# razvanmatisan/duodiff

Hardware: AMD Instinct MI355X
Metric: images/sec (whole node) DuoDiff 1000-step CelebA-64 (higher is better)
Workload: dtype bf16

## Files before the change

duodiff_amd/csrc/attention.hip:

```cpp
#include "dd_internal.h"

#include <type_traits>
#include <utility>

namespace dd {
namespace {

constexpr int kMaxKeyTiles = 9;
constexpr int kLP = kMaxKeyTiles * 32;
constexpr int kHD = 64;
constexpr int kPartBytes = 4 * 2 * 66 * 4;

__device__ __forceinline__ unsigned pack2_bf16(float lo, float hi) {
    typedef __bf16 bf16v2 __attribute__((ext_vector_type(2)));
    typedef float f32v2 __attribute__((ext_vector_type(2)));
    const f32v2 q = {lo, hi};
    return __builtin_bit_cast(unsigned, __builtin_convertvector(q, bf16v2));
}

__device__ __forceinline__ unsigned lds_addr_of(const void* p) {
    return (unsigned)(size_t)(const __attribute__((address_space(3))) char*)p;
}

__device__ __forceinline__ int k_swz(int r) { return ((r >> 1) & 7) ^ ((r & 1) << 2); }
__device__ __forceinline__ int v_swz(int r) { return (2 * (r & 3)) ^ ((r >> 2) & 1); }

template <typename T> struct AttnLayout;
template <> struct AttnLayout<bf16_t> {
    static constexpr int kRowK = 128;
    static constexpr int kRowV = 128;
    static constexpr int kVBytes = kLP * kRowV;
};
template <> struct AttnLayout<float> {
    static constexpr int kRowK = 256 + 16;
    static constexpr int kRowV = kLP * 4 + 16;
    static constexpr int kVBytes = kHD * kRowV;
};

template <typename T, int NKT, int NT, bool KPERM, typename TileFn>
__device__ __forceinline__ void attend_tiles(const char* Ks, const char* Vt, int L, int nkt, int lane, TileFn&& tile,
                                         const f32x4 (&qcur)[sizeof(T) == 2 ? 4 : 8], f32x16 (&o)[2], float& mx, float& sum) {
    using Lay = AttnLayout<T>;
    const int half = lane >> 5, r32 = lane & 31;
    const f32x16 zero16 = {0.f, 0.f, 0.f, 0.f, 0.f, 0.f, 0.f, 0.f, 0.f, 0.f, 0.f, 0.f, 0.f, 0.f, 0.f, 0.f};
    f32x16 s[NT];

    if constexpr (sizeof(T) == 2) {
        bf16x8 qf[4];
#pragma unroll
        for (int st = 0; st < 4; ++st) qf[st] = __builtin_bit_cast(bf16x8, qcur[st]);
        auto load_k = [&](int t, bf16x8 (&kf)[4]) {
            const char* kr = Ks + (t * 32 + r32) * Lay::kRowK;
            const int sw = k_swz(r32);
#pragma unroll
            for (int st = 0; st < 4; ++st) {
                const int ch = KPERM ? 4 * (st >> 1) + 2 * half + (st & 1) : 2 * st + half;
                kf[st] = *reinterpret_cast<const bf16x8*>(kr + ((ch ^ sw) << 4));
            }
        };
        bf16x8 kfa[4], kfb[4];
        if (tile(0) >= 0) load_k(tile(0), kfa);
#pragma unroll
        for (int k = 0; k < NT; ++k) {
            const int t = tile(k);
            const int tn = k + 1 < NT ? tile(k + 1) : -1;
            if (tn >= 0) { if (k & 1) load_k(tn, kfa); else load_k(tn, kfb); }
            __builtin_amdgcn_sched_barrier(0);
            if (t >= 0) {
                s[k] = __builtin_amdgcn_mfma_f32_32x32x16_bf16((k & 1) ? kfb[0] : kfa[0], qf[0], zero16, 0, 0, 0);
#pragma unroll
                for (int st = 1; st < 4; ++st)
                    s[k] = __builtin_amdgcn_mfma_f32_32x32x16_bf16((k & 1) ? kfb[st] : kfa[st], qf[st], s[k], 0, 0, 0);
            } else {
                s[k] = zero16;
            }
            __builtin_amdgcn_sched_barrier(0);
        }
    } else {
#pragma unroll
        for (int k = 0; k < NT; ++k) {
            const int t = tile(k);
            s[k] = zero16;
            if (t >= 0) {
                const char* kr = Ks + (t * 32 + r32) * Lay::kRowK + (32 * half) * 4;
#pragma unroll
                for (int g = 0; g < 8; ++g) {
                    const f32x4 kf = *reinterpret_cast<const f32x4*>(kr + g * 16);
#pragma unroll
                    for (int e = 0; e < 4; ++e)
                        s[k] = __builtin_amdgcn_mfma_f32_32x32x2f32(kf[e], qcur[g][e], s[k], 0, 0, 0);
                }
            }
        }
    }

    mx = -INFINITY;
#pragma unroll
    for (int k = 0; k < NT; ++k) {
        const int t = tile(k);
        if (t >= 0) {
            if (t == nkt - 1) {
#pragma unroll
                for (int e = 0; e < 16; ++e) {
                    const int key = t * 32 + (e & 3) + 8 * (e >> 2) + 4 * half;
                    if (key >= L) s[k][e] = -INFINITY;
                }
            }
#pragma unroll
            for (int e = 0; e < 16; ++e) mx = fmaxf(mx, s[k][e]);
        }
    }
    mx = fmaxf(mx, __shfl_xor(mx, 32));
    constexpr float kScaleLog2e = 0.125f * 1.4426950408889634f;
    const float mxs = mx * kScaleLog2e;
    sum = 0.f;
#pragma unroll
    for (int k = 0; k < NT; ++k) {
        if (tile(k) >= 0) {
#pragma unroll
            for (int e = 0; e < 16; ++e) {
                float p;
                if (NKT == 9 && NT == 9 && k == 8 && e >= 2) {
                    s[k][e] = 0.f;
                    continue;
                }
                if constexpr (sizeof(T) == 2) p = __builtin_amdgcn_exp2f(fmaf(s[k][e], kScaleLog2e, -mxs));
                else p = expf((s[k][e] - mx) * 0.125f);
                s[k][e] = p;
                sum += p;
            }
        }
    }
    sum += __shfl_xor(sum, 32);

    o[0] = zero16;
    o[1] = zero16;

    if constexpr (sizeof(T) == 2) {
        typedef __attribute__((ext_vector_type(4))) short s4;
        struct VF { s4 lo[2][2], hi[2][2]; };
        const int tq = (lane >> 2) & 3, tp = lane & 3, dhalf = (lane >> 4) & 1;
        const char* vb0 = Vt + (4 * half + tq) * Lay::kRowV + 8 * (tp & 1);
        const int vsw = v_swz(4 * half + tq);
        const char* vbd[2] = {vb0 + (((2 * dhalf + (tp >> 1)) ^ vsw) << 4), vb0 + (((4 + 2 * dhalf + (tp >> 1)) ^ vsw) << 4)};
        typedef __attribute__((address_space(3))) s4* lds_s4_ptr;
        auto load_v = [&](int t, VF& f) {
#pragma unroll
            for (int st = 0; st < 2; ++st)
#pragma unroll
                for (int dt = 0; dt < 2; ++dt) {
                    const char* vr = vbd[dt] + (t * 32 + 16 * st) * Lay::kRowV;
                    f.lo[st][dt] = __builtin_amdgcn_ds_read_tr16_b64_v4i16((lds_s4_ptr)(size_t)lds_addr_of(vr));
                    f.hi[st][dt] = __builtin_amdgcn_ds_read_tr16_b64_v4i16((lds_s4_ptr)(size_t)lds_addr_of(vr + 8 * Lay::kRowV));
                }
        };
        VF va, vb;
        if (tile(0) >= 0) load_v(tile(0), va);
#pragma unroll
        for (int k = 0; k < NT; ++k) {
            const int t = tile(k);
            const int tn = k + 1 < NT ? tile(k + 1) : -1;
            if (tn >= 0) { if (k & 1) load_v(tn, va); else load_v(tn, vb); }
            __builtin_amdgcn_sched_barrier(0);
            if (t >= 0) {
                const VF& f = (k & 1) ? vb : va;
#pragma unroll
                for (int st = 0; st < 2; ++st) {
                    bf16x8 pf;
#pragma unroll
                    for (int j = 0; j < 8; ++j) pf[j] = (short)f2bf(s[k][8 * st + j]);
#pragma unroll
                    for (int dt = 0; dt < 2; ++dt) {
                        bf16x8 vf;
#pragma unroll
                        for (int j = 0; j < 4; ++j) { vf[j] = f.lo[st][dt][j]; vf[4 + j] = f.hi[st][dt][j]; }
                        o[dt] = __builtin_amdgcn_mfma_f32_32x32x16_bf16(vf, pf, o[dt], 0, 0, 0);
                    }
                }
            }
            __builtin_amdgcn_sched_barrier(0);
        }
    } else {
#pragma unroll
        for (int k = 0; k < NT; ++k) {
            const int t = tile(k);
            if (t >= 0) {
#pragma unroll
                for (int g = 0; g < 4; ++g) {
#pragma unroll
                    for (int dt = 0; dt < 2; ++dt) {
                        const char* vr = Vt + (dt * 32 + r32) * Lay::kRowV + (t * 32 + 8 * g + 4 * half) * 4;
                        const f32x4 vf = *reinterpret_cast<const f32x4*>(vr);
#pragma unroll
                        for (int e = 0; e < 4; ++e)
                            o[dt] = __builtin_amdgcn_mfma_f32_32x32x2f32(vf[e], s[k][4 * g + e], o[dt], 0, 0, 0);
                    }
                }
            }
        }
    }
}

template <typename T, int NKT>
__global__ void __launch_bounds__(256, sizeof(T) == 2 ? 2 : 1)
attention_kernel(const T* __restrict__ qkv, T* __restrict__ out, int B, int L, int H, int D, int Lp) {
    using Lay = AttnLayout<T>;
    extern __shared__ __attribute__((aligned(16))) char smem[];
    char* Ks = smem;
    char* Vt = smem + kLP * Lay::kRowK;

    const int b = blockIdx.x / H, hh = blockIdx.x % H;
    const int tid = threadIdx.x, lane = tid & 63, wave = tid >> 6;
    const int half = lane >> 5, r32 = lane & 31;
    constexpr long long ld = kHD;
    const long long unit = (long long)Lp * kHD;
    const T* qbase = qkv + ((long long)b * 3 * H + hh) * unit;
    const T* kbase = qbase + (long long)H * unit;
    const T* vbase = kbase + (long long)H * unit;
    const int nkt = NKT > 0 ? NKT : (L + 31) / 32;
    constexpr int EPC = 16 / (int)sizeof(T);
    constexpr int CPR = kHD / EPC;

    constexpr int NQF = sizeof(T) == 2 ? 4 : 8;
    auto load_q = [&](int qc, f32x4 (&qf)[NQF]) {
        const int q = qc * 32 + r32;
        const T* qrow = qbase + (long long)(q < L ? q : L - 1) * ld;
#pragma unroll
        for (int i = 0; i < NQF; ++i)
            qf[i] = sizeof(T) == 2 ? *reinterpret_cast<const f32x4*>(qrow + 16 * i + 8 * half)
                                   : *reinterpret_cast<const f32x4*>(qrow + 32 * half + 4 * i);
    };
    f32x4 qnext[NQF];
    load_q(wave, qnext);

    if constexpr (sizeof(T) == 2) {
        typedef const __attribute__((address_space(1))) void* gptr_t;
        typedef __attribute__((address_space(3))) void* lptr_t;
        const int np = Lp >> 3;
        const int wv = __builtin_amdgcn_readfirstlane(wave);
        const int lr = lane >> 3, slot = lane & 7;
        constexpr int MAXP = (kLP / 8 * 2 + 3) / 4;
#pragma unroll
        for (int i = 0; i < MAXP; ++i) {
            const int p2 = wv + 4 * i;
            if (p2 < 2 * np) {
                const bool isv = p2 >= np;
                const int p = isv ? p2 - np : p2, r = 8 * p + lr;
                const int ch = isv ? (slot ^ v_swz(r)) : (slot ^ k_swz(r));
                const T* src = (isv ? vbase : kbase) + (long long)(r < L ? r : L - 1) * kHD + ch * 8;
                char* dst = (isv ? Vt : Ks) + p * 1024;
                __builtin_amdgcn_global_load_lds((gptr_t)src, (lptr_t)dst, 16, 0, 0);
            }
        }
        for (int i = tid; i < (nkt * 32 - Lp) * 16; i += 256) {
            const int rr = Lp + (i >> 4), c = i & 15;
            *reinterpret_cast<f32x4*>((c < 8 ? Ks : Vt) + rr * 128 + (c & 7) * 16) = f32x4{0.f, 0.f, 0.f, 0.f};
        }
        asm volatile("s_waitcnt vmcnt(0)" ::: "memory");
    } else {
        for (int idx = tid; idx < nkt * 32 * CPR; idx += 256) {
            const int key = idx / CPR, ch = idx % CPR;
            f32x4 kv = {0.f, 0.f, 0.f, 0.f}, vv = {0.f, 0.f, 0.f, 0.f};
            if (key < L) {
                kv = *reinterpret_cast<const f32x4*>(kbase + (long long)key * ld + ch * EPC);
                vv = *reinterpret_cast<const f32x4*>(vbase + (long long)key * ld + ch * EPC);
            }
            *reinterpret_cast<f32x4*>(Ks + key * Lay::kRowK + ch * 16) = kv;
            T tmp[EPC];
            *reinterpret_cast<f32x4*>(tmp) = vv;
#pragma unroll
            for (int e = 0; e < EPC; ++e)
                *reinterpret_cast<T*>(Vt + (ch * EPC + e) * Lay::kRowV + key * (int)sizeof(T)) = tmp[e];
        }
    }

    __syncthreads();

    constexpr bool SPLIT_LAST = NKT == 9;
    const int nqc = (L + 31) / 32;
    const int n_regular = SPLIT_LAST ? 8 : nqc;
    for (int qc = wave; qc < n_regular; qc += 4) {
        const int q = qc * 32 + r32;
        f32x4 qcur[NQF];
#pragma unroll
        for (int i = 0; i < NQF; ++i) qcur[i] = qnext[i];
        if (qc + 4 < n_regular) load_q(qc + 4, qnext);
        else if (SPLIT_LAST) load_q(8, qnext);

        f32x16 o[2];
        float mx, sum;
        attend_tiles<T, NKT, kMaxKeyTiles, false>(Ks, Vt, L, nkt, lane, [&](int k) { return k < nkt ? k : -1; }, qcur, o, mx, sum);
        const float inv = 1.0f / sum;

        T* orow = out + ((long long)b * L + (q < L ? q : L - 1)) * D + hh * kHD;
        if constexpr (sizeof(T) == 2) {
#pragma unroll
            for (int dt = 0; dt < 2; ++dt) {
                uint2 v[4];
#pragma unroll
                for (int g = 0; g < 4; ++g) {
                    bf16_t v4[4];
#pragma unroll
                    for (int e = 0; e < 4; ++e) v4[e] = f2bf(o[dt][4 * g + e] * inv);
                    v[g] = *reinterpret_cast<const uint2*>(v4);
                }
#pragma unroll
                for (int gp = 0; gp < 4; gp += 2) {
                    const auto s0 = __builtin_amdgcn_permlane32_swap(v[gp].x, v[gp + 1].x, false, false);
                    const auto s1 = __builtin_amdgcn_permlane32_swap(v[gp].y, v[gp + 1].y, false, false);
                    const uint4 o4 = {s0[0], s1[0], s0[1], s1[1]};
                    if (q < L) *reinterpret_cast<uint4*>(orow + dt * 32 + 8 * gp + 8 * half) = o4;
                }
            }
        } else if (q < L) {
#pragma unroll
            for (int dt = 0; dt < 2; ++dt)
#pragma unroll
                for (int g = 0; g < 4; ++g) {
                    const int d = dt * 32 + 8 * g + 4 * half;
                    *reinterpret_cast<f32x4*>(orow + d) = f32x4{o[dt][4 * g] * inv, o[dt][4 * g + 1] * inv, o[dt][4 * g + 2] * inv, o[dt][4 * g + 3] * inv};
                }
        }
    }

    if constexpr (SPLIT_LAST) {
        float* part = reinterpret_cast<float*>(smem + kLP * Lay::kRowK + Lay::kVBytes);
        const int rem = L - 256;
        f32x16 o[2];
        float mx, sum;
        attend_tiles<T, NKT, 3, false>(Ks, Vt, L, nkt, lane, [&](int k) { return k < 2 ? wave + 4 * k : (wave == 3 ? 8 : -1); }, qnext, o, mx, sum);
        if (r32 < rem) {
            float* pw = part + (wave * 2 + r32) * 66;
#pragma unroll
            for (int dt = 0; dt < 2; ++dt)
#pragma unroll
                for (int g = 0; g < 4; ++g)
                    *reinterpret_cast<f32x4*>(pw + dt * 32 + 8 * g + 4 * half) =
                        f32x4{o[dt][4 * g], o[dt][4 * g + 1], o[dt][4 * g + 2], o[dt][4 * g + 3]};
            if (half == 0) { pw[64] = mx; pw[65] = sum; }
        }
        __syncthreads();
        if (tid < rem * 64) {
            const int qi = tid >> 6, d = tid & 63;
            float m[4], M = -INFINITY;
#pragma unroll
            for (int w = 0; w < 4; ++w) { m[w] = part[(w * 2 + qi) * 66 + 64]; M = fmaxf(M, m[w]); }
            float num = 0.f, den = 0.f;
#pragma unroll
            for (int w = 0; w < 4; ++w) {
                float f;
                if constexpr (sizeof(T) == 2) f = __builtin_amdgcn_exp2f((m[w] - M) * (0.125f * 1.4426950408889634f));
                else f = expf((m[w] - M) * 0.125f);
                num = fmaf(f, part[(w * 2 + qi) * 66 + d], num);
                den = fmaf(f, part[(w * 2 + qi) * 66 + 65], den);
            }
            out[((long long)b * L + 256 + qi) * D + hh * kHD + d] = Elem<T>::from_f32(num / den);
        }
    }
}


struct QkvAttnArgs {
    const bf16_t* h;
    const bf16_t* wimg;
    const float* bias;
    const bf16_t* hx;
    const float* xres;
    const float* ln_g;
    const float* ln_b;
    bf16_t* out;
    int B, L, H, Lp, E;
};

constexpr int kQaPxBytes = 8 * 6 * 2 * 32 * 4;
constexpr int kQaHxPad = 64;
constexpr int kQaHxBytes = 2 * (1024 * 2 + kQaHxPad);
constexpr int kQaAuxBytes = kQaPxBytes + kQaHxBytes + 256;
constexpr int kQaKQ = 8;
constexpr int kQaBlk = 2 * kQaKQ * 1024;
constexpr int kQaRing = 4 * kQaBlk;
static_assert(8 * 2 * 66 * 4 <= kQaPxBytes, "the split chunk's partials reuse the px area");

typedef const __attribute__((address_space(1))) void* qa_gptr_t;
typedef __attribute__((address_space(3))) void* qa_lptr_t;

constexpr int qa_dma_ops(int b, int nb) { return b < nb ? 2 : 0; }
constexpr int qa_pref_ops(int b, int nb) { return (b >= 0 && b % 3 == 0 && b / 3 + 1 < nb / 3) ? kQaKQ : 0; }
constexpr int qa_younger_dma(int b, int nb) { return qa_pref_ops(b - 1, nb) + qa_dma_ops(b + 2, nb) + qa_pref_ops(b, nb); }
constexpr int qa_younger_rows(int b, int nb) { return qa_dma_ops(b, nb) + qa_dma_ops(b + 1, nb) + qa_dma_ops(b + 2, nb); }

template <int D>
__global__ void __launch_bounds__(512, 1) qkv_attention_kernel(const QkvAttnArgs a) {
    using Lay = AttnLayout<bf16_t>;
    constexpr int KS = D / 16, NS = KS / kQaKQ, NB = 3 * NS;
    static_assert(D % 128 == 0 && D >= 512 && D <= 1024, "k range in slices of 8 k-steps; hxl holds two rows of D <= 1024");
    extern __shared__ __attribute__((aligned(16))) char smem[];
    char* Ks = smem;
    char* Vt = smem + kLP * Lay::kRowK;
    float* px = reinterpret_cast<float*>(smem + kLP * Lay::kRowK + Lay::kVBytes);
    float* part = px;
    char* hxl = smem + kLP * Lay::kRowK + Lay::kVBytes + kQaPxBytes;
    char* qxl = hxl + kQaHxBytes;
    char* ring = smem + kLP * Lay::kRowK + Lay::kVBytes + kQaAuxBytes;

    int b, hh;
    if ((a.B & 7) == 0) { const int slot = blockIdx.x >> 3; b = (blockIdx.x & 7) + 8 * (slot / a.H); hh = slot % a.H; }
    else { b = blockIdx.x / a.H; hh = blockIdx.x % a.H; }
    const int tid = threadIdx.x, lane = tid & 63, wave = __builtin_amdgcn_readfirstlane(tid >> 6);
    const int half = lane >> 5, r32 = lane & 31;
    const int L = a.L, E = a.E;

    const char* wsrc = reinterpret_cast<const char*>(a.wimg) + (size_t)hh * NB * kQaBlk;
    const unsigned lane16 = lane * 16;
    auto dma_block = [&](int bb) {
#pragma unroll
        for (int i = 0; i < 2; ++i) {
            const int pc = wave * 2 + i;
            const char* sb = wsrc + (size_t)bb * kQaBlk + pc * 1024;
            const unsigned lds = lds_addr_of(ring + (bb & 3) * kQaBlk + pc * 1024);
            asm volatile("s_mov_b32 m0, %0\n\tglobal_load_lds_dwordx4 %1, %2" ::"s"(lds), "v"(lane16), "s"(sb) : "memory", "m0");
        }
    };
    dma_block(0);
    dma_block(1);
    dma_block(2);

    const int row = 32 * wave + r32;
    const bf16x8* hfr_u = reinterpret_cast<const bf16x8*>(a.h) + ((long long)b * 8 + wave) * KS * 64;
    const bf16x8* hfr = hfr_u + lane;
    bf16x8 xs[2][kQaKQ];
#pragma unroll
    for (int ks = 0; ks < kQaKQ; ++ks) xs[0][ks] = hfr[ks * 64];

    if (a.hx) {
        for (int i = tid; i < E * (D / 8); i += 512) {
            const int e = i / (D / 8), cch = i % (D / 8);
            *reinterpret_cast<f32x4*>(hxl + e * (D * 2 + kQaHxPad) + cch * 16) = *reinterpret_cast<const f32x4*>(a.hx + ((long long)b * L + e) * D + cch * 8);
        }
    } else if (wave < E) {
        constexpr int NV = D / 256;
        const float* xr = a.xres + ((long long)b * L + wave) * D + lane * (D / 64);
        f32x4 xv[NV];
        float s1 = 0.f;
#pragma unroll
        for (int v = 0; v < NV; ++v) {
            xv[v] = *reinterpret_cast<const f32x4*>(xr + 4 * v);
            s1 += (xv[v][0] + xv[v][1]) + (xv[v][2] + xv[v][3]);
        }
#pragma unroll
        for (int o = 32; o >= 1; o >>= 1) s1 += __shfl_xor(s1, o);
        const float mean = s1 / (float)D;
        float s2 = 0.f;
#pragma unroll
        for (int v = 0; v < NV; ++v) {
            xv[v] = xv[v] - mean;
            s2 += (xv[v][0] * xv[v][0] + xv[v][1] * xv[v][1]) + (xv[v][2] * xv[v][2] + xv[v][3] * xv[v][3]);
        }
#pragma unroll
        for (int o = 32; o >= 1; o >>= 1) s2 += __shfl_xor(s2, o);
        const float rstd = 1.0f / sqrtf(s2 / (float)D + 1e-5f);
#pragma unroll
        for (int v = 0; v < NV; ++v) {
            const f32x4 g = *reinterpret_cast<const f32x4*>(a.ln_g + lane * (D / 64) + 4 * v), c0 = *reinterpret_cast<const f32x4*>(a.ln_b + lane * (D / 64) + 4 * v);
            const f32x4 y = xv[v] * rstd * g + c0;
            *reinterpret_cast<uint2*>(hxl + wave * (D * 2 + kQaHxPad) + (lane * (D / 64) + 4 * v) * 2) = uint2{pack2_bf16(y[0], y[1]), pack2_bf16(y[2], y[3])};
        }
    }
    for (int i = tid; i < (kLP - 256 - E) * 16; i += 512) {
        const int r = 256 + E + (i >> 4), c = i & 15;
        *reinterpret_cast<f32x4*>((c < 8 ? Ks : Vt) + r * 128 + (c & 7) * 16) = f32x4{0.f, 0.f, 0.f, 0.f};
    }

    const f32x16 zero16 = {0.f, 0.f, 0.f, 0.f, 0.f, 0.f, 0.f, 0.f, 0.f, 0.f, 0.f, 0.f, 0.f, 0.f, 0.f, 0.f};
    f32x16 acc[6];
#pragma unroll
    for (int j = 0; j < 6; ++j) acc[j] = zero16;
    f32x4 accx[6];
#pragma unroll
    for (int j = 0; j < 6; ++j) accx[j] = f32x4{0.f, 0.f, 0.f, 0.f};
    const int xg = lane >> 4, xn = lane & 15;
    const int wx16 = (2 * (wave >> 1) + (xg >> 1)) * 1024 + ((16 * (wave & 1) + xn) + 32 * (xg & 1)) * 16;
    const char* hx16 = hxl + (xn < E ? xn : 0) * (D * 2 + kQaHxPad) + (wave >> 1) * 64 + xg * 16;
    bf16x8 wq[4];
    asm volatile("s_waitcnt vmcnt(0)\n\ts_waitcnt lgkmcnt(0)\n\ts_barrier" ::: "memory");
#pragma unroll
    for (int i = 0; i < 4; ++i) wq[i] = *reinterpret_cast<const bf16x8*>(ring + lane * 16 + i * 1024);
    [&]<int... BI>(std::integer_sequence<int, BI...>) {
        ([&] {
            constexpr int bb = BI, q = bb / 3, jj = bb % 3, S = q & 1;
            if constexpr (jj == 0) {
                if constexpr (q > 0) {
                    asm volatile("s_waitcnt vmcnt(%8)"
                                 : "+v"(xs[S][0]), "+v"(xs[S][1]), "+v"(xs[S][2]), "+v"(xs[S][3]), "+v"(xs[S][4]), "+v"(xs[S][5]), "+v"(xs[S][6]), "+v"(xs[S][7])
                                 : "i"(qa_younger_rows(bb, NB)));
                }
                if constexpr (q + 1 < NS) {
#pragma unroll
                    for (int ks = 0; ks < kQaKQ; ++ks)
                        asm volatile("global_load_dwordx4 %0, %1, %2" : "=v"(xs[S ^ 1][ks]) : "v"(lane16), "s"(hfr_u + ((q + 1) * kQaKQ + ks) * 64) : "memory");
                }
            }
            const char* wb = ring + (bb & 3) * kQaBlk + lane * 16;
            const char* wbn = ring + ((bb + 1) & 3) * kQaBlk + lane * 16;
#pragma unroll
            for (int f = 0; f < 2 * kQaKQ; ++f) {
                if (f == kQaKQ) {
                    if constexpr (bb + 1 < NB) {
                        if constexpr (bb + 1 >= 3) asm volatile("s_waitcnt vmcnt(%0)\n\ts_barrier" ::"i"(qa_younger_dma(bb, NB)) : "memory");
                        else asm volatile("s_barrier" ::: "memory");
                    }
                    if constexpr (bb + 3 < NB) dma_block(bb + 3);
                    const bf16x8 hb = *reinterpret_cast<const bf16x8*>(hx16 + q * (kQaKQ * 32));
#pragma unroll
                    for (int t = 0; t < 2; ++t) {
                        const bf16x8 wa = *reinterpret_cast<const bf16x8*>(ring + (bb & 3) * kQaBlk + t * (kQaKQ * 1024) + wx16);
                        accx[2 * jj + t] = __builtin_amdgcn_mfma_f32_16x16x32_bf16(wa, hb, accx[2 * jj + t], 0, 0, 0);
                    }
                }
                const bf16x8 w0 = wq[f & 3];
                if (f + 4 < 2 * kQaKQ) wq[f & 3] = *reinterpret_cast<const bf16x8*>(wb + (f + 4) * 1024);
                else if (bb + 1 < NB) wq[f & 3] = *reinterpret_cast<const bf16x8*>(wbn + (f + 4 - 2 * kQaKQ) * 1024);
                acc[2 * jj + (f >> 3)] = __builtin_amdgcn_mfma_f32_32x32x16_bf16(w0, xs[S][f & 7], acc[2 * jj + (f >> 3)], 0, 0, 0);
            }
        }(), ...);
    }(std::make_integer_sequence<int, NB>{});

    if (xn < E) {
#pragma unroll
        for (int j = 0; j < 6; ++j) *reinterpret_cast<f32x4*>(px + (((wave * 6 + j) * 2 + xn) * 16 + 4 * xg)) = accx[j];
    }
    f32x4 qcur[4];
    const int swk = k_swz(row), swv = v_swz(row);
#pragma unroll
    for (int j = 0; j < 6; ++j) {
        if (a.bias) {
            const float* bj = a.bias + (j >> 1) * D + hh * kHD + 32 * (j & 1) + 4 * half;
#pragma unroll
            for (int g = 0; g < 4; ++g) {
                const f32x4 bv = *reinterpret_cast<const f32x4*>(bj + 8 * g);
#pragma unroll
                for (int e = 0; e < 4; ++e) acc[j][4 * g + e] += bv[e];
            }
        }
        unsigned pk[8];
#pragma unroll
        for (int i = 0; i < 8; ++i) pk[i] = pack2_bf16(acc[j][2 * i], acc[j][2 * i + 1]);
        const int T = j & 1;
        if (j < 2) {
            qcur[2 * T] = __builtin_bit_cast(f32x4, uint4{pk[0], pk[1], pk[2], pk[3]});
            qcur[2 * T + 1] = __builtin_bit_cast(f32x4, uint4{pk[4], pk[5], pk[6], pk[7]});
        } else if (j < 4) {
            *reinterpret_cast<uint4*>(Ks + row * 128 + (((4 * T + 2 * half) ^ swk) << 4)) = uint4{pk[0], pk[1], pk[2], pk[3]};
            *reinterpret_cast<uint4*>(Ks + row * 128 + (((4 * T + 2 * half + 1) ^ swk) << 4)) = uint4{pk[4], pk[5], pk[6], pk[7]};
        } else {
#pragma unroll
            for (int gp = 0; gp < 4; gp += 2) {
                const auto s0 = __builtin_amdgcn_permlane32_swap(pk[2 * gp], pk[2 * gp + 2], false, false);
                const auto s1 = __builtin_amdgcn_permlane32_swap(pk[2 * gp + 1], pk[2 * gp + 3], false, false);
                *reinterpret_cast<uint4*>(Vt + row * 128 + (((4 * T + gp + half) ^ swv) << 4)) = uint4{s0[0], s1[0], s0[1], s1[1]};
            }
        }
    }
    __syncthreads();
    if (tid < E * 192) {
        const int e = tid / 192, c = tid % 192, j = c >> 5, col = c & 31;
        float v = a.bias ? a.bias[(j >> 1) * D + hh * kHD + 32 * (j & 1) + col] : 0.f;
#pragma unroll
        for (int kb = 0; kb < 4; ++kb) v += px[(((2 * kb + (col >> 4)) * 6 + j) * 2 + e) * 16 + (col & 15)];
        const bf16_t vb = f2bf(v);
        const int d = 32 * (j & 1) + col, r = 256 + e;
        if (j < 2) {
            *reinterpret_cast<bf16_t*>(qxl + e * 128 + d * 2) = vb;
        } else if (j < 4) {
            const int T = d >> 5, dd = d & 31, hf = (dd >> 2) & 1, ae = (dd & 3) + 4 * (dd >> 3);
            *reinterpret_cast<bf16_t*>(Ks + r * 128 + (((4 * T + 2 * hf + (ae >> 3)) ^ k_swz(r)) << 4) + (ae & 7) * 2) = vb;
        } else {
            *reinterpret_cast<bf16_t*>(Vt + r * 128 + (((d >> 3) ^ v_swz(r)) << 4) + (d & 7) * 2) = vb;
        }
    }
    __syncthreads();

    f32x4 qe[4];
    {
        const bf16_t* qrow = reinterpret_cast<const bf16_t*>(qxl) + (r32 < E ? r32 : E - 1) * kHD + 4 * half;
#pragma unroll
        for (int st = 0; st < 4; ++st) {
            const uint2 lo = *reinterpret_cast<const uint2*>(qrow + 32 * (st >> 1) + 16 * (st & 1));
            const uint2 hi = *reinterpret_cast<const uint2*>(qrow + 32 * (st >> 1) + 16 * (st & 1) + 8);
            qe[st] = __builtin_bit_cast(f32x4, uint4{lo.x, lo.y, hi.x, hi.y});
        }
    }

    {
        f32x16 o[2];
        float mx, sum;
        attend_tiles<bf16_t, 9, kMaxKeyTiles, true>(Ks, Vt, L, kMaxKeyTiles, lane, [&](int k) { return k; }, qcur, o, mx, sum);
        const float inv = 1.0f / sum;
        bf16_t* orow = a.out + ((long long)b * L + E + row) * D + hh * kHD;
#pragma unroll
        for (int dt = 0; dt < 2; ++dt) {
            uint2 v[4];
#pragma unroll
            for (int g = 0; g < 4; ++g) {
                bf16_t v4[4];
#pragma unroll
                for (int e = 0; e < 4; ++e) v4[e] = f2bf(o[dt][4 * g + e] * inv);
                v[g] = *reinterpret_cast<const uint2*>(v4);
            }
#pragma unroll
            for (int gp = 0; gp < 4; gp += 2) {
                const auto s0 = __builtin_amdgcn_permlane32_swap(v[gp].x, v[gp + 1].x, false, false);
                const auto s1 = __builtin_amdgcn_permlane32_swap(v[gp].y, v[gp + 1].y, false, false);
                *reinterpret_cast<uint4*>(orow + dt * 32 + 8 * gp + 8 * half) = uint4{s0[0], s1[0], s0[1], s1[1]};
            }
        }
    }

    {
        f32x16 o[2];
        float mx, sum;
        attend_tiles<bf16_t, 9, 2, true>(Ks, Vt, L, kMaxKeyTiles, lane, [&](int k) { return k == 0 ? wave : (wave == 7 ? 8 : -1); }, qe, o, mx, sum);
        if (r32 < E) {
            float* pw = part + (wave * 2 + r32) * 66;
#pragma unroll
            for (int dt = 0; dt < 2; ++dt)
#pragma unroll
                for (int g = 0; g < 4; ++g)
                    *reinterpret_cast<f32x4*>(pw + dt * 32 + 8 * g + 4 * half) =
                        f32x4{o[dt][4 * g], o[dt][4 * g + 1], o[dt][4 * g + 2], o[dt][4 * g + 3]};
            if (half == 0) { pw[64] = mx; pw[65] = sum; }
        }
        __syncthreads();
        if (tid < E * 64) {
            const int qi = tid >> 6, d = tid & 63;
            float m[8], M = -INFINITY;
#pragma unroll
            for (int w = 0; w < 8; ++w) { m[w] = part[(w * 2 + qi) * 66 + 64]; M = fmaxf(M, m[w]); }
            float num = 0.f, den = 0.f;
#pragma unroll
            for (int w = 0; w < 8; ++w) {
                const float f = __builtin_amdgcn_exp2f((m[w] - M) * (0.125f * 1.4426950408889634f));
                num = fmaf(f, part[(w * 2 + qi) * 66 + d], num);
                den = fmaf(f, part[(w * 2 + qi) * 66 + 65], den);
            }
            a.out[((long long)b * L + qi) * D + hh * kHD + d] = f2bf(num / den);
        }
    }
}

}

template <typename T>
hipError_t launch_attention(const T* qkv, T* out, int B, int L, int H, int D, hipStream_t s) {
    if (L > kLP || D != H * kHD || L < 1) return hipErrorInvalidValue;
    using Lay = AttnLayout<T>;
    const size_t lds = (size_t)kLP * Lay::kRowK + (size_t)Lay::kVBytes + kPartBytes;
    const int Lp = make_head_major(L, H).Lp;
    if (L == 257 || L == 258) hipLaunchKernelGGL((attention_kernel<T, 9>), dim3(B * H), dim3(256), lds, s, qkv, out, B, L, H, D, Lp);
    else hipLaunchKernelGGL((attention_kernel<T, 0>), dim3(B * H), dim3(256), lds, s, qkv, out, B, L, H, D, Lp);
    return hipGetLastError();
}

void qkv_attention_pack(int D, int H, const float* w, unsigned short (*to_bf16)(float), unsigned short* img) {
    const int NS = D / 16 / kQaKQ;
    for (int hh = 0; hh < H; ++hh)
        for (int q = 0; q < NS; ++q)
            for (int j = 0; j < 6; ++j)
                for (int ks = 0; ks < kQaKQ; ++ks)
                    for (int lane = 0; lane < 64; ++lane) {
                        const float* src = w + ((size_t)(j >> 1) * D + 64 * hh + 32 * (j & 1) + (lane & 31)) * D + 16 * (q * kQaKQ + ks) + 8 * (lane >> 5);
                        unsigned short* dst = img + (((((size_t)hh * NS + q) * 6 + j) * kQaKQ + ks) * 64 + lane) * 8;
                        for (int i = 0; i < 8; ++i) dst[i] = to_bf16(src[i]);
                    }
}

bool qkv_attention_supported(int D, int H, int L, int extras) {
    return (D == 512 || D == 768 || D == 1024) && H * kHD == D && (extras == 1 || extras == 2) && L == 256 + extras;
}

static size_t qkv_attention_lds() { return (size_t)kLP * AttnLayout<bf16_t>::kRowK + AttnLayout<bf16_t>::kVBytes + kQaAuxBytes + kQaRing; }

hipError_t launch_qkv_attention(const bf16_t* h, const bf16_t* wimg, const float* bias, const bf16_t* hx, const float* xres,
                                const float* ln_g, const float* ln_b, bf16_t* out, int B, int L, int H, int D, int extras, hipStream_t s) {
    if (!qkv_attention_supported(D, H, L, extras) || !h || !wimg || (!hx && (!xres || !ln_g || !ln_b)) || !out || B < 1) return hipErrorInvalidValue;
    const QkvAttnArgs a{h, wimg, bias, hx, xres, ln_g, ln_b, out, B, L, H, make_head_major(L, H).Lp, extras};
    switch (D) {
        case 512: hipLaunchKernelGGL((qkv_attention_kernel<512>), dim3(B * H), dim3(512), qkv_attention_lds(), s, a); break;
        case 768: hipLaunchKernelGGL((qkv_attention_kernel<768>), dim3(B * H), dim3(512), qkv_attention_lds(), s, a); break;
        default: hipLaunchKernelGGL((qkv_attention_kernel<1024>), dim3(B * H), dim3(512), qkv_attention_lds(), s, a); break;
    }
    return hipGetLastError();
}

hipError_t init_attention_kernels() {
    for (const void* f : {(const void*)qkv_attention_kernel<512>, (const void*)qkv_attention_kernel<768>, (const void*)qkv_attention_kernel<1024>})
        if (hipError_t e = hipFuncSetAttribute(f, hipFuncAttributeMaxDynamicSharedMemorySize, (int)qkv_attention_lds()); e != hipSuccess) return e;
    const int lb = kLP * AttnLayout<bf16_t>::kRowK + AttnLayout<bf16_t>::kVBytes + kPartBytes;
    const int lf = kLP * AttnLayout<float>::kRowK + AttnLayout<float>::kVBytes + kPartBytes;
    hipError_t e = hipFuncSetAttribute((const void*)attention_kernel<bf16_t, 9>, hipFuncAttributeMaxDynamicSharedMemorySize, lb);
    if (e == hipSuccess) e = hipFuncSetAttribute((const void*)attention_kernel<bf16_t, 0>, hipFuncAttributeMaxDynamicSharedMemorySize, lb);
    if (e == hipSuccess) e = hipFuncSetAttribute((const void*)attention_kernel<float, 9>, hipFuncAttributeMaxDynamicSharedMemorySize, lf);
    if (e == hipSuccess) e = hipFuncSetAttribute((const void*)attention_kernel<float, 0>, hipFuncAttributeMaxDynamicSharedMemorySize, lf);
    return e;
}

template hipError_t launch_attention<bf16_t>(const bf16_t*, bf16_t*, int, int, int, int, hipStream_t);
template hipError_t launch_attention<float>(const float*, float*, int, int, int, int, hipStream_t);

}
```

Measured before the change: 47.93.

## Interleave softmax max/exp with QK and PV MFMA loops in bf16 attention

In the bf16 attention path, the row-max reduction for each key tile now runs inside the QK^T MFMA loop, one tile behind. The exp and bf16 packing for the next tile runs inside the PV MFMA loop, and sched_group_barrier hints interleave VALU work with MFMAs. Cross-half reductions use permlane32_swap instead of shfl_xor, and an s_nop is added after the m0 write before global_load_lds. This aims to hide softmax VALU latency behind matrix work, at the cost of more live registers (pf for all tiles), which may cause spills or lower occupancy.

```diff
diff --git a/duodiff_amd/csrc/attention.hip b/duodiff_amd/csrc/attention.hip
--- a/duodiff_amd/csrc/attention.hip
+++ b/duodiff_amd/csrc/attention.hip
@@ -58,6 +58,20 @@
                 kf[st] = *reinterpret_cast<const bf16x8*>(kr + ((ch ^ sw) << 4));
             }
         };
+        mx = -INFINITY;
+        auto tile_max = [&](int k) {
+            const int t = tile(k);
+            if (t < 0) return;
+            if (t == nkt - 1) {
+#pragma unroll
+                for (int e = 0; e < 16; ++e) {
+                    const int key = t * 32 + (e & 3) + 8 * (e >> 2) + 4 * half;
+                    if (key >= L) s[k][e] = -INFINITY;
+                }
+            }
+#pragma unroll
+            for (int e = 0; e < 16; ++e) mx = fmaxf(mx, s[k][e]);
+        };
         bf16x8 kfa[4], kfb[4];
         if (tile(0) >= 0) load_k(tile(0), kfa);
 #pragma unroll
@@ -74,69 +88,44 @@
             } else {
                 s[k] = zero16;
             }
+            if (k > 0) tile_max(k - 1);
+#pragma unroll
+            for (int g = 0; g < 4; ++g) {
+                __builtin_amdgcn_sched_group_barrier(0x008, 1, 0);
+                __builtin_amdgcn_sched_group_barrier(0x002, 4, 0);
+            }
             __builtin_amdgcn_sched_barrier(0);
         }
-    } else {
-#pragma unroll
-        for (int k = 0; k < NT; ++k) {
-            const int t = tile(k);
-            s[k] = zero16;
-            if (t >= 0) {
-                const char* kr = Ks + (t * 32 + r32) * Lay::kRowK + (32 * half) * 4;
-#pragma unroll
-                for (int g = 0; g < 8; ++g) {
-                    const f32x4 kf = *reinterpret_cast<const f32x4*>(kr + g * 16);
-#pragma unroll
-                    for (int e = 0; e < 4; ++e)
-                        s[k] = __builtin_amdgcn_mfma_f32_32x32x2f32(kf[e], qcur[g][e], s[k], 0, 0, 0);
-                }
-            }
-        }
-    }
-
-    mx = -INFINITY;
-#pragma unroll
-    for (int k = 0; k < NT; ++k) {
-        const int t = tile(k);
-        if (t >= 0) {
-            if (t == nkt - 1) {
-#pragma unroll
-                for (int e = 0; e < 16; ++e) {
-                    const int key = t * 32 + (e & 3) + 8 * (e >> 2) + 4 * half;
-                    if (key >= L) s[k][e] = -INFINITY;
-                }
-            }
-#pragma unroll
-            for (int e = 0; e < 16; ++e) mx = fmaxf(mx, s[k][e]);
-        }
-    }
-    mx = fmaxf(mx, __shfl_xor(mx, 32));
-    constexpr float kScaleLog2e = 0.125f * 1.4426950408889634f;
-    const float mxs = mx * kScaleLog2e;
-    sum = 0.f;
-#pragma unroll
-    for (int k = 0; k < NT; ++k) {
-        if (tile(k) >= 0) {
+        tile_max(NT - 1);
+        {
+            const auto x = __builtin_amdgcn_permlane32_swap(__float_as_uint(mx), __float_as_uint(mx), false, false);
+            mx = fmaxf(__uint_as_float(x[0]), __uint_as_float(x[1]));
+        }
+
+        constexpr float kScaleLog2e = 0.125f * 1.4426950408889634f;
+        const float mxs = mx * kScaleLog2e;
+        sum = 0.f;
+        bf16x8 pf[NT][2];
+        auto tile_exp = [&](int k) {
+            if (tile(k) < 0) return;
 #pragma unroll
             for (int e = 0; e < 16; ++e) {
-                float p;
                 if (NKT == 9 && NT == 9 && k == 8 && e >= 2) {
                     s[k][e] = 0.f;
                     continue;
                 }
-                if constexpr (sizeof(T) == 2) p = __builtin_amdgcn_exp2f(fmaf(s[k][e], kScaleLog2e, -mxs));
-                else p = expf((s[k][e] - mx) * 0.125f);
+                const float p = __builtin_amdgcn_exp2f(fmaf(s[k][e], kScaleLog2e, -mxs));
                 s[k][e] = p;
                 sum += p;
             }
-        }
-    }
-    sum += __shfl_xor(sum, 32);
-
-    o[0] = zero16;
-    o[1] = zero16;
-
-    if constexpr (sizeof(T) == 2) {
+#pragma unroll
+            for (int st = 0; st < 2; ++st)
+#pragma unroll
+                for (int j = 0; j < 8; ++j) pf[k][st][j] = (short)f2bf(s[k][8 * st + j]);
+        };
+
+        o[0] = zero16;
+        o[1] = zero16;
         typedef __attribute__((ext_vector_type(4))) short s4;
         struct VF { s4 lo[2][2], hi[2][2]; };
         const int tq = (lane >> 2) & 3, tp = lane & 3, dhalf = (lane >> 4) & 1;
@@ -156,6 +145,7 @@
         };
         VF va, vb;
         if (tile(0) >= 0) load_v(tile(0), va);
+        tile_exp(0);
 #pragma unroll
         for (int k = 0; k < NT; ++k) {
             const int t = tile(k);
@@ -165,22 +155,79 @@
             if (t >= 0) {
                 const VF& f = (k & 1) ? vb : va;
 #pragma unroll
-                for (int st = 0; st < 2; ++st) {
-                    bf16x8 pf;
-#pragma unroll
-                    for (int j = 0; j < 8; ++j) pf[j] = (short)f2bf(s[k][8 * st + j]);
+                for (int st = 0; st < 2; ++st)
 #pragma unroll
                     for (int dt = 0; dt < 2; ++dt) {
                         bf16x8 vf;
 #pragma unroll
                         for (int j = 0; j < 4; ++j) { vf[j] = f.lo[st][dt][j]; vf[4 + j] = f.hi[st][dt][j]; }
-                        o[dt] = __builtin_amdgcn_mfma_f32_32x32x16_bf16(vf, pf, o[dt], 0, 0, 0);
+                        o[dt] = __builtin_amdgcn_mfma_f32_32x32x16_bf16(vf, pf[k][st], o[dt], 0, 0, 0);
                     }
-                }
+            }
+            if (k + 1 < NT) tile_exp(k + 1);
+#pragma unroll
+            for (int g = 0; g < 4; ++g) {
+                __builtin_amdgcn_sched_group_barrier(0x008, 1, 0);
+                __builtin_amdgcn_sched_group_barrier(0x002, 14, 0);
             }
             __builtin_amdgcn_sched_barrier(0);
         }
+        {
+            const auto x = __builtin_amdgcn_permlane32_swap(__float_as_uint(sum), __float_as_uint(sum), false, false);
+            sum = __uint_as_float(x[0]) + __uint_as_float(x[1]);
+        }
     } else {
+#pragma unroll
+        for (int k = 0; k < NT; ++k) {
+            const int t = tile(k);
+            s[k] = zero16;
+            if (t >= 0) {
+                const char* kr = Ks + (t * 32 + r32) * Lay::kRowK + (32 * half) * 4;
+#pragma unroll
+                for (int g = 0; g < 8; ++g) {
+                    const f32x4 kf = *reinterpret_cast<const f32x4*>(kr + g * 16);
+#pragma unroll
+                    for (int e = 0; e < 4; ++e)
+                        s[k] = __builtin_amdgcn_mfma_f32_32x32x2f32(kf[e], qcur[g][e], s[k], 0, 0, 0);
+                }
+            }
+        }
+        mx = -INFINITY;
+#pragma unroll
+        for (int k = 0; k < NT; ++k) {
+            const int t = tile(k);
+            if (t >= 0) {
+                if (t == nkt - 1) {
+#pragma unroll
+                    for (int e = 0; e < 16; ++e) {
+                        const int key = t * 32 + (e & 3) + 8 * (e >> 2) + 4 * half;
+                        if (key >= L) s[k][e] = -INFINITY;
+                    }
+                }
+#pragma unroll
+                for (int e = 0; e < 16; ++e) mx = fmaxf(mx, s[k][e]);
+            }
+        }
+        mx = fmaxf(mx, __shfl_xor(mx, 32));
+        sum = 0.f;
+#pragma unroll
+        for (int k = 0; k < NT; ++k) {
+            if (tile(k) >= 0) {
+#pragma unroll
+                for (int e = 0; e < 16; ++e) {
+                    if (NKT == 9 && NT == 9 && k == 8 && e >= 2) {
+                        s[k][e] = 0.f;
+                        continue;
+                    }
+                    const float p = expf((s[k][e] - mx) * 0.125f);
+                    s[k][e] = p;
+                    sum += p;
+                }
+            }
+        }
+        sum += __shfl_xor(sum, 32);
+        o[0] = zero16;
+        o[1] = zero16;
 #pragma unroll
         for (int k = 0; k < NT; ++k) {
             const int t = tile(k);
@@ -418,7 +465,7 @@
             const int pc = wave * 2 + i;
             const char* sb = wsrc + (size_t)bb * kQaBlk + pc * 1024;
             const unsigned lds = lds_addr_of(ring + (bb & 3) * kQaBlk + pc * 1024);
-            asm volatile("s_mov_b32 m0, %0\n\tglobal_load_lds_dwordx4 %1, %2" ::"s"(lds), "v"(lane16), "s"(sb) : "memory", "m0");
+            asm volatile("s_mov_b32 m0, %0\n\ts_nop 0\n\tglobal_load_lds_dwordx4 %1, %2" ::"s"(lds), "v"(lane16), "s"(sb) : "memory", "m0");
         }
     };
     dma_block(0);
```

Result: no change. 47.81 (median of 6 runs) (-0.2%).
